# p2004dr/visual-slam

Measured on AMD Instinct MI355X. Metric: frames/sec (extract+match+pose) at 640×480, 2000 ORB, 1/2/4/8 MI355X, higher is better.
Workload: dtype u8

## Files before the change

visual-slam_amd/csrc/twoview_kernels.hip:

```cpp
#include <cmath>

#include "common.h"

#define TV_BLOCK 256
typedef double v4d __attribute__((ext_vector_type(4)));
#define TVF_BLOCK 512

#define TV_PARTS 4
#define TV_REC 10

struct TvWork {
    double* xn;
    float* xf;
    float* px;
    int* qidx;
    uint8_t* cbits;
    int* m;
    double* surv;
    int* n_alive;
    int* n_tasks;
    int2* task;
    unsigned long long* wkey;
    double* wE;
    unsigned long long* best;
// ... 257 lines not shown
}

__device__ __forceinline__ double sampson_fast(const double* E, double x1, double y1, double x2, double y2) {
    const double ex0 = fma(E[0], x1, fma(E[1], y1, E[2]));
    const double ex1 = fma(E[3], x1, fma(E[4], y1, E[5]));
    const double ex2 = fma(E[6], x1, fma(E[7], y1, E[8]));
    const double et0 = fma(E[0], x2, fma(E[3], y2, E[6]));
    const double et1 = fma(E[1], x2, fma(E[4], y2, E[7]));
    const double num = fma(x2, ex0, fma(y2, ex1, ex2));
    const double den = fma(ex0, ex0, fma(ex1, ex1, fma(et0, et0, et1 * et1)));
    double r = (double)__builtin_amdgcn_rcpf((float)den);
    r = fma(fma(-den, r, 1.0), r, r);
    return num * num * r;
}

__device__ inline uint64_t splitmix64(uint64_t& s) {
    uint64_t z = (s += 0x9E3779B97F4A7C15ull);
    z = (z ^ (z >> 30)) * 0xBF58476D1CE4E5B9ull;
    z = (z ^ (z >> 27)) * 0x94D049BB133111EBull;
    return z ^ (z >> 31);
}

__device__ __forceinline__ void sample8(uint64_t seed, int h, int m, int (&idx)[8]) {
    const uint32_t um = (uint32_t)m, q0 = 0xFFFFFFFFu / um, r0 = 0xFFFFFFFFu - q0 * um;
    const uint32_t M = r0 + 1u == um ? q0 + 1u : q0, c32 = r0 + 1u == um ? 0u : r0 + 1u;
    const bool small = m <= 65536;
    auto mod32 = [um, M](uint32_t x) {
        uint32_t r = x - __umulhi(x, M) * um;
        return r >= um ? r - um : r;
    };
    uint64_t s = seed + (uint64_t)(h + 1) * 0xD1B54A32D192ED03ull;
#pragma unroll
    for (int k = 0; k < 8; k++) {
        int c;
        bool dup;
        do {
            const uint64_t z = splitmix64(s);
            c = small ? (int)mod32(mod32((uint32_t)(z >> 32)) * c32 + mod32((uint32_t)z)) : (int)(z % (uint64_t)um);
            dup = false;
#pragma unroll
            for (int j = 0; j < k; j++) dup |= idx[j] == c;
        } while (dup);
        idx[k] = c;
    }
}

__device__ bool eight_point(const double* pts , double* E) {
    double M[9][8];
#pragma unroll
    for (int k = 0; k < 8; k++) {
        double x1 = pts[k * 4], y1 = pts[k * 4 + 1], x2 = pts[k * 4 + 2], y2 = pts[k * 4 + 3];
        M[0][k] = x2 * x1; M[1][k] = x2 * y1; M[2][k] = x2;
        M[3][k] = y2 * x1; M[4][k] = y2 * y1; M[5][k] = y2;
        M[6][k] = x1;      M[7][k] = y1;      M[8][k] = 1.0;
    }
    double beta[8];
    bool ok = true;
#pragma unroll
    for (int k = 0; k < 8; k++) {
        double nrm2 = 0;
#pragma unroll
        for (int i = k; i < 9; i++) nrm2 += M[i][k] * M[i][k];
        double nrm = sqrt(nrm2);
        ok = ok && (nrm > 1e-13);
        double alpha = M[k][k] >= 0 ? -nrm : nrm;
        double v0 = M[k][k] - alpha;
        M[k][k] = v0;
        double vtv = nrm2 - 2.0 * alpha * (v0 + alpha) + alpha * alpha;
        vtv = vtv > 0 ? vtv : 1.0;
        beta[k] = 2.0 / vtv;
#pragma unroll
        for (int j = k + 1; j < 8; j++) {
            double dot = 0;
#pragma unroll
            for (int i = k; i < 9; i++) dot += M[i][k] * M[i][j];
            dot *= beta[k];
#pragma unroll
            for (int i = k; i < 9; i++) M[i][j] -= dot * M[i][k];
        }
    }
    double n[9] = {0, 0, 0, 0, 0, 0, 0, 0, 1.0};
#pragma unroll
    for (int k = 7; k >= 0; k--) {
        double dot = 0;
#pragma unroll
        for (int i = k; i < 9; i++) dot += M[i][k] * n[i];
        dot *= beta[k];
#pragma unroll
        for (int i = k; i < 9; i++) n[i] -= dot * M[i][k];
    }
    double nn = 0;
#pragma unroll
    for (int j = 0; j < 9; j++) nn += n[j] * n[j];
    nn = 1.0 / sqrt(nn);
#pragma unroll
    for (int j = 0; j < 9; j++) E[j] = n[j] * nn;
    return ok;
}

__device__ __forceinline__ double tv_thr(const TwoViewArgs& a, const TvWork& w, int pair) {
    return a.model ? a.thr_px * w.norm[(size_t)pair * 8] : a.thr_px / ((a.K[0] + a.K[4]) / 2.0);
}

__device__ bool project_rank2(double* F) {
    double v[3];
    if (!smallest_right3(F, v)) return false;
    for (int i = 0; i < 3; i++) {
        const double fv = F[i * 3] * v[0] + F[i * 3 + 1] * v[1] + F[i * 3 + 2] * v[2];
        for (int j = 0; j < 3; j++) F[i * 3 + j] -= fv * v[j];
    }
    return true;
}

__device__ void tv_hartley(const TwoViewArgs& a, const TvWork& w, int pair, int m) {
    __shared__ double s_h[TV_BLOCK / 64][5];
    __shared__ double s_nrm[5];
    const int tid = threadIdx.x;
    const float* px = w.px + (size_t)pair * a.cap * 4;
    double* xn = w.xn + (size_t)pair * a.cap * 4;
    __syncthreads();
    double acc[4] = {0, 0, 0, 0};
    for (int i = tid; i < m; i += TV_BLOCK)
        for (int k = 0; k < 4; k++) acc[k] += (double)px[4 * i + k];
    for (int k = 0; k < 4; k++) {
        for (int o = 32; o > 0; o >>= 1) acc[k] += __shfl_xor(acc[k], o, 64);
        if ((tid & 63) == 0) s_h[tid >> 6][k] = acc[k];
    }
    __syncthreads();
    if (tid < 4) s_nrm[1 + tid] = (s_h[0][tid] + s_h[1][tid] + s_h[2][tid] + s_h[3][tid]) / (double)max(m, 1);
    __syncthreads();
    const double c1x = s_nrm[1], c1y = s_nrm[2], c2x = s_nrm[3], c2y = s_nrm[4];
    double dsum = 0;
    for (int i = tid; i < m; i += TV_BLOCK) {
        const double a1 = (double)px[4 * i] - c1x, b1 = (double)px[4 * i + 1] - c1y, a2 = (double)px[4 * i + 2] - c2x, b2 = (double)px[4 * i + 3] - c2y;
        dsum += sqrt(a1 * a1 + b1 * b1) + sqrt(a2 * a2 + b2 * b2);
    }
    for (int o = 32; o > 0; o >>= 1) dsum += __shfl_xor(dsum, o, 64);
    if ((tid & 63) == 0) s_h[tid >> 6][4] = dsum;
    __syncthreads();
    if (tid == 0) {
        const double mean = (s_h[0][4] + s_h[1][4] + s_h[2][4] + s_h[3][4]) / (2.0 * (double)max(m, 1));
        s_nrm[0] = mean > 1e-12 ? 1.4142135623730951 / mean : 1.0;
        double* o = w.norm + (size_t)pair * 8;
        o[0] = s_nrm[0]; o[1] = c1x; o[2] = c1y; o[3] = c2x; o[4] = c2y;
    }
    __syncthreads();
    const double sc = s_nrm[0];
    for (int i = tid; i < m; i += TV_BLOCK) {
        xn[4 * i] = sc * ((double)px[4 * i] - c1x); xn[4 * i + 1] = sc * ((double)px[4 * i + 1] - c1y);
        xn[4 * i + 2] = sc * ((double)px[4 * i + 2] - c2x); xn[4 * i + 3] = sc * ((double)px[4 * i + 3] - c2y);
    }
}

__device__ void tv_f32_copy(const TwoViewArgs& a, const TvWork& w, int pair, int m) {
    __shared__ float s_mx[TV_BLOCK / 64];
    const int tid = threadIdx.x;
    const double* xn = w.xn + (size_t)pair * a.cap * 4;
    float* xf = w.xf + (size_t)pair * a.cap * 4;
    __syncthreads();
    float mx = 1.0f;
    for (int i = tid; i < 4 * m; i += TV_BLOCK) {
        const float v = (float)xn[i];
        xf[i] = v;
        mx = fmaxf(mx, fabsf(v));
    }
    for (int o = 32; o > 0; o >>= 1) mx = fmaxf(mx, __shfl_xor(mx, o, 64));
    if ((tid & 63) == 0) s_mx[tid >> 6] = mx;
    __syncthreads();
    if (tid == 0) w.norm[(size_t)pair * 8 + 5] = (double)fmaxf(fmaxf(s_mx[0], s_mx[1]), fmaxf(s_mx[2], s_mx[3])) * 1.0000002;
}

__global__ __launch_bounds__(TV_BLOCK) void k_tv_prep(TwoViewArgs a, TvWork w) {
    const int pair = blockIdx.x, tid = threadIdx.x;
    __shared__ int s_w[TV_BLOCK / 64];
    __shared__ int s_base;
    const double fx = a.K[0], fy = a.K[4], cx = a.K[2], cy = a.K[5];
    double* xn = w.xn + (size_t)pair * a.cap * 4;
    float* px = w.px + (size_t)pair * a.cap * 4;
    int* qidx = w.qidx + (size_t)pair * a.cap;
    if (tid == 0) {
        s_base = 0; w.best[pair] = ~0ull; w.n_alive[pair] = 0; if (pair == 0) *w.n_tasks = 0;
        *(unsigned*)&w.norm[(size_t)pair * 8 + 6] = 0x7F800000u;
    }
    for (int j = tid; j < (a.n_hyp + 63) / 64; j += TV_BLOCK) w.wkey[(size_t)pair * ((a.n_hyp + 63) / 64) + j] = ~0ull;
    __syncthreads();
    if (a.d_p1) {
        int m = a.m_fixed;
        for (int i = tid; i < m; i += TV_BLOCK) {
            float u1 = a.d_p1[(size_t)pair * m * 2 + 2 * i], v1 = a.d_p1[(size_t)pair * m * 2 + 2 * i + 1];
            float u2 = a.d_p2[(size_t)pair * m * 2 + 2 * i], v2 = a.d_p2[(size_t)pair * m * 2 + 2 * i + 1];
            px[4 * i] = u1; px[4 * i + 1] = v1; px[4 * i + 2] = u2; px[4 * i + 3] = v2;
            xn[4 * i] = ((double)u1 - cx) / fx; xn[4 * i + 1] = ((double)v1 - cy) / fy;
            xn[4 * i + 2] = ((double)u2 - cx) / fx; xn[4 * i + 3] = ((double)v2 - cy) / fy;
            qidx[i] = i;
        }
        if (tid == 0) w.m[pair] = m;
        if (a.model) tv_hartley(a, w, pair, m);
        tv_f32_copy(a, w, pair, m);
        return;
    }
    const int qfr = a.d_qf ? a.d_qf[pair] : pair, tfr = a.d_tf ? a.d_tf[pair] : pair + 1;
    const mo_keypoint* k1 = a.d_kps + (size_t)qfr * a.cap;
    const mo_keypoint* k2 = a.d_kps + (size_t)tfr * a.cap;
    if (a.d_sel) {
        const int m = min(a.d_sel_n[pair], a.cap);
        const int32_t* sl = a.d_sel + (size_t)pair * a.cap * 2;
        for (int o = tid; o < m; o += TV_BLOCK) {
            const int i = sl[2 * o], j = sl[2 * o + 1];
            float u1 = k1[i].x, v1 = k1[i].y, u2 = k2[j].x, v2 = k2[j].y;
            px[4 * o] = u1; px[4 * o + 1] = v1; px[4 * o + 2] = u2; px[4 * o + 3] = v2;
            xn[4 * o] = ((double)u1 - cx) / fx; xn[4 * o + 1] = ((double)v1 - cy) / fy;
            xn[4 * o + 2] = ((double)u2 - cx) / fx; xn[4 * o + 3] = ((double)v2 - cy) / fy;
            qidx[o] = i;
        }
        if (tid == 0) w.m[pair] = m;
        if (a.model) tv_hartley(a, w, pair, m);
        tv_f32_copy(a, w, pair, m);
        return;
    }
    const int nq = min(a.d_counts[qfr], a.cap);
    const int32_t* midx = a.d_match_idx + (size_t)pair * a.cap * 2;
    const uint8_t* pass = a.d_match_pass + (size_t)pair * a.cap;
    for (int base = 0; base < nq; base += TV_BLOCK) {
        int i = base + tid;
        bool ok = i < nq && pass[i] && (!a.need_two || midx[2 * i + 1] >= 0);
        unsigned long long bal = __ballot(ok);
        int lane = tid & 63, wv = tid >> 6;
        int wpre = __popcll(bal & ((1ull << lane) - 1ull));
        if (lane == 0) s_w[wv] = __popcll(bal);
        __syncthreads();
        int off = s_base;
        for (int k = 0; k < wv; k++) off += s_w[k];
        if (ok) {
            int o = off + wpre;
            int j = midx[2 * i];
            float u1 = k1[i].x, v1 = k1[i].y, u2 = k2[j].x, v2 = k2[j].y;
            px[4 * o] = u1; px[4 * o + 1] = v1; px[4 * o + 2] = u2; px[4 * o + 3] = v2;
            xn[4 * o] = ((double)u1 - cx) / fx; xn[4 * o + 1] = ((double)v1 - cy) / fy;
            xn[4 * o + 2] = ((double)u2 - cx) / fx; xn[4 * o + 3] = ((double)v2 - cy) / fy;
            qidx[o] = i;
        }
        __syncthreads();
        if (tid == 0) s_base += s_w[0] + s_w[1] + s_w[2] + s_w[3];
        __syncthreads();
    }
    const int m = s_base;
    if (tid == 0) w.m[pair] = m;
    if (a.model) tv_hartley(a, w, pair, m);
    tv_f32_copy(a, w, pair, m);
}


#ifndef TV_FIRST_NUM
#define TV_FIRST_NUM 2
#endif
__device__ __forceinline__ int tv_first(int m, int num) { return min(m, max(32, (m * num + 7) >> 3)); }

__device__ __forceinline__ int tv_part_len(int m) { return (m + TV_PARTS - 1) / TV_PARTS; }
__device__ __forceinline__ double tv_cost_part(const double* E, const double* xn, int i0, int i1, double thr2) {
    typedef const __attribute__((address_space(4))) double* cdp;
    const cdp pts = (cdp)(uintptr_t)xn;
    double s = 0.0;
#pragma unroll 4
    for (int i = i0; i < i1; i++) s += fmin(sampson_fast(E, pts[4 * i], pts[4 * i + 1], pts[4 * i + 2], pts[4 * i + 3]), thr2);
    return s;
}
__device__ __forceinline__ double tv_combine(const double (&P)[TV_PARTS]) { return (P[0] + P[1]) + (P[2] + P[3]); }
__device__ __forceinline__ double tv_cost_lane(const double* E, const double* xn, int m, double thr2) {
    const int q = tv_part_len(m);
    double P[TV_PARTS];
    for (int k = 0; k < TV_PARTS; k++) P[k] = tv_cost_part(E, xn, min(m, k * q), min(m, (k + 1) * q), thr2);
    return tv_combine(P);
}

__global__ __launch_bounds__(TV_BLOCK) void k_tv_hyp(TwoViewArgs a, TvWork w, int staged, int first_num) {
    __shared__ unsigned long long s_best[TV_BLOCK / 64];
    const int pair = blockIdx.y, hb = blockIdx.x, tid = threadIdx.x;
    const int h = hb * TV_BLOCK + tid;
    const int m = w.m[pair];
    if (m < 8) return;
    const double* xn = w.xn + (size_t)pair * a.cap * 4;
    const double thr = tv_thr(a, w, pair);
    const double thr2 = thr * thr;
    double E[9];
    bool valid = h < a.n_hyp;
    if (valid) {
        int idx[8];
        sample8(a.seed + ((uint64_t)pair + a.pair_base) * 0x632BE59BD9B4E019ull, h, m, idx);
        double pts[32];
        for (int k = 0; k < 8; k++)
            for (int j = 0; j < 4; j++) pts[k * 4 + j] = xn[(size_t)idx[k] * 4 + j];
        valid = eight_point(pts, E) && (a.model ? project_rank2(E) : project_essential(E));
    }
    if (!valid) for (int j = 0; j < 9; j++) E[j] = 0.0;
    const int lane = tid & 63, wv = tid >> 6;
    const size_t ntask_max = (size_t)((a.n_hyp + 63) / 64);
    unsigned long long key = ~0ull;
    if (!staged) {
        const double cost = valid ? tv_cost_lane(E, xn, m, thr2) : 0.0;
        if (valid && cost == cost) key = ((unsigned long long)__float_as_uint((float)cost) << 32) | (unsigned long long)(unsigned)h;
        const unsigned long long own = key;
        for (int o = 32; o > 0; o >>= 1) {
            unsigned long long other = __shfl_xor(key, o, 64);
            key = other < key ? other : key;
        }
        if (lane == 0) s_best[wv] = key;
        __syncthreads();
        for (int k = 0; k < TV_BLOCK / 64; k++) key = s_best[k] < key ? s_best[k] : key;
        if (key != ~0ull && own == key) {
            double* bE = w.wE + ((size_t)pair * ntask_max + hb) * 9;
            for (int j = 0; j < 9; j++) bE[j] = E[j];
            w.wkey[(size_t)pair * ntask_max + hb] = key;
            atomicMin(&w.best[pair], key);
        }
        return;
    }
    typedef const __attribute__((address_space(4))) float* cfp;
    const cfp pf = (cfp)(uintptr_t)(w.xf + (size_t)pair * a.cap * 4);
    const int F = tv_first(m, first_num);
    const float X = (float)w.norm[(size_t)pair * 8 + 5];
    float lb = 0.0f;
    if (valid && X < 1e6f) {
        float e[9], s1 = 0.0f;
        for (int j = 0; j < 9; j++) { e[j] = (float)E[j]; s1 += fabsf(e[j]); }
        s1 *= 1.000001f;
        const float ae = 4e-7f * X * s1, delta = 2e-6f * X * X * s1, cden = 4004.0f * ae * ae;
        const float thr2f = __uint_as_float(__float_as_uint((float)thr2) - 1u);
#pragma unroll 4
        for (int i = 0; i < F; i++) {
            const float x1 = pf[4 * i], y1 = pf[4 * i + 1], x2 = pf[4 * i + 2], y2 = pf[4 * i + 3];
            const float ex0 = fmaf(e[0], x1, fmaf(e[1], y1, e[2]));
            const float ex1 = fmaf(e[3], x1, fmaf(e[4], y1, e[5]));
            const float ex2 = fmaf(e[6], x1, fmaf(e[7], y1, e[8]));
            const float et0 = fmaf(e[0], x2, fmaf(e[3], y2, e[6]));
            const float et1 = fmaf(e[1], x2, fmaf(e[4], y2, e[7]));
            const float r = fmaf(x2, ex0, fmaf(y2, ex1, ex2));
            const float den = fmaf(ex0, ex0, fmaf(ex1, ex1, fmaf(et0, et0, et1 * et1)));
            const float rl = fmaxf(fabsf(r) - delta, 0.0f);
            const float t = rl * rl * __builtin_amdgcn_rcpf(fmaf(den, 1.0011f, cden));
            lb += fminf(t, thr2f);
        }
        lb *= 0.9999f;
        if (!(lb >= 0.0f)) lb = 0.0f;
    }
    if (valid) key = ((unsigned long long)__float_as_uint(lb) << 32) | (unsigned long long)(unsigned)h;
    const unsigned long long own = key;
    for (int o = 32; o > 0; o >>= 1) {
        unsigned long long other = __shfl_xor(key, o, 64);
        key = other < key ? other : key;
    }
    if (lane == 0) s_best[wv] = key;
    __syncthreads();
    for (int k = 0; k < TV_BLOCK / 64; k++) key = s_best[k] < key ? s_best[k] : key;
    if (key == ~0ull) return;
    __shared__ double s_cand[9];
    __shared__ double s_sum[TV_BLOCK / 64];
    __shared__ unsigned s_bound;
    if (own == key)
        for (int j = 0; j < 9; j++) s_cand[j] = E[j];
    __syncthreads();
    {
        double Ec[9];
        for (int j = 0; j < 9; j++) Ec[j] = s_cand[j];
        double tot = 0.0;
        for (int i = tid; i < m; i += TV_BLOCK)
            tot += fmin(sampson_fast(Ec, xn[4 * i], xn[4 * i + 1], xn[4 * i + 2], xn[4 * i + 3]), thr2);
        for (int o = 32; o > 0; o >>= 1) tot += __shfl_xor(tot, o, 64);
        if (lane == 0) s_sum[wv] = tot;
    }
    __syncthreads();
    if (tid == 0) {
        double total = 0.0;
        for (int k = 0; k < TV_BLOCK / 64; k++) total += s_sum[k];
        unsigned bound = total == total ? __float_as_uint((float)total) + 2u : 0x7F800000u;
        const unsigned seen = atomicMin((unsigned*)&w.norm[(size_t)pair * 8 + 6], bound);
        s_bound = min(bound, seen);
    }
    __syncthreads();
    __shared__ int s_wcnt[TV_BLOCK / 64];
    __shared__ int s_gbase;
    const bool alive = own != ~0ull && __float_as_uint(lb) <= s_bound;
    const unsigned long long mk = __ballot(alive);
    if (lane == 0) s_wcnt[wv] = __popcll(mk);
    __syncthreads();
    int sbase = 0, n_alive = 0;
    for (int k = 0; k < TV_BLOCK / 64; k++) { if (k < wv) sbase += s_wcnt[k]; n_alive += s_wcnt[k]; }
    if (tid == 0) s_gbase = atomicAdd(&w.n_alive[pair], n_alive);
    __syncthreads();
    if (alive) {
        double* rec = w.surv + ((size_t)pair * a.n_hyp + s_gbase + sbase + __popcll(mk & ((1ull << lane) - 1ull))) * TV_REC;
        for (int j = 0; j < 9; j++) rec[j] = E[j];
        rec[9] = __longlong_as_double((long long)h);
    }
}

__global__ __launch_bounds__(TV_BLOCK) void k_tv_tasks(TwoViewArgs a, TvWork w) {
    __shared__ int s_off[TV_BLOCK + 1];
    const int tid = threadIdx.x;
    int total = 0;
    for (int p0 = 0; p0 < a.n_pairs; p0 += TV_BLOCK) {
        const int p = p0 + tid;
        const int nt = p < a.n_pairs ? (w.n_alive[p] + 63) / 64 : 0;
        s_off[tid + 1] = nt;
        __syncthreads();
        if (tid == 0) {
            s_off[0] = total;
            for (int k = 0; k < TV_BLOCK; k++) s_off[k + 1] += s_off[k];
        }
        __syncthreads();
        for (int j = 0; j < nt; j++) w.task[s_off[tid] + j] = make_int2(p, j);
        total = s_off[TV_BLOCK];
        __syncthreads();
    }
    if (tid == 0) *w.n_tasks = total;
}

__global__ __launch_bounds__(64 * TV_PARTS) void k_tv_score(TwoViewArgs a, TvWork w, int one_pair) {
    __shared__ double s_part[TV_PARTS][64];
    const int lane = threadIdx.x & 63, part = threadIdx.x >> 6;
    if (one_pair ? (int)blockIdx.x * 64 >= w.n_alive[0] : (int)blockIdx.x >= *w.n_tasks) return;
    const int2 tk = one_pair ? make_int2(0, (int)blockIdx.x) : w.task[blockIdx.x];
    const int pair = tk.x, t0 = tk.y * 64;
    const int total = w.n_alive[pair];
    const int m = w.m[pair];
    const double thr = tv_thr(a, w, pair);
    const double thr2 = thr * thr;
    const double* xn = w.xn + (size_t)pair * a.cap * 4;
    const bool on = t0 + lane < total;
    const double* rec = w.surv + ((size_t)pair * a.n_hyp + (on ? t0 + lane : t0)) * TV_REC;
    double E[9];
    for (int j = 0; j < 9; j++) E[j] = rec[j];
    const int q = tv_part_len(m);
    s_part[part][lane] = tv_cost_part(E, xn, min(m, part * q), min(m, (part + 1) * q), thr2);
    __syncthreads();
    if (part != 0) return;
    double P[TV_PARTS];
    for (int k = 0; k < TV_PARTS; k++) P[k] = s_part[k][lane];
    const double cost = tv_combine(P);
    const unsigned h = (unsigned)__double_as_longlong(rec[9]);
    unsigned long long key = ~0ull;
    if (on && cost == cost) key = ((unsigned long long)__float_as_uint((float)cost) << 32) | (unsigned long long)h;
    const unsigned long long own = key;
    for (int o = 32; o > 0; o >>= 1) {
        unsigned long long other = __shfl_xor(key, o, 64);
        key = other < key ? other : key;
    }
    if (key != ~0ull && own == key) {
        const size_t slot = (size_t)pair * ((a.n_hyp + 63) / 64) + tk.y;
        for (int j = 0; j < 9; j++) w.wE[slot * 9 + j] = E[j];
        w.wkey[slot] = key;
        atomicMin(&w.best[pair], key);
    }
}

#define DLT_VOTE_IT 8
#define DLT_MAP_IT 32
__device__ void dlt_point(const double* P1, const double* P2, double x1, double y1, double x2, double y2, double* X, int max_it) {
    double A[16];
#pragma unroll
    for (int k = 0; k < 4; k++) {
        A[0 * 4 + k] = x1 * P1[8 + k] - P1[k];
        A[1 * 4 + k] = y1 * P1[8 + k] - P1[4 + k];
        A[2 * 4 + k] = x2 * P2[8 + k] - P2[k];
        A[3 * 4 + k] = y2 * P2[8 + k] - P2[4 + k];
    }
    double S[10];
#pragma unroll
    for (int i = 0, k = 0; i < 4; i++)
#pragma unroll
        for (int j = i; j < 4; j++, k++) S[k] = A[i] * A[j] + A[4 + i] * A[4 + j] + A[8 + i] * A[8 + j] + A[12 + i] * A[12 + j];
    X[0] = 0.5; X[1] = 0.5; X[2] = 0.5; X[3] = 0.5;
    smallest_eigvec<4>(S, X, max_it);
}

__device__ inline double block_sum(double v, double* s_red) {
    for (int o = 32; o > 0; o >>= 1) v += __shfl_xor(v, o, 64);
    __syncthreads();
    if ((threadIdx.x & 63) == 0) s_red[threadIdx.x >> 6] = v;
    __syncthreads();
    double r = 0;
    for (int k = 0; k < TVF_BLOCK / 64; k++) r += s_red[k];
    return r;
}

__device__ inline int block_sum_i(int v, int* s_red) {
    for (int o = 32; o > 0; o >>= 1) v += __shfl_xor(v, o, 64);
    __syncthreads();
    if ((threadIdx.x & 63) == 0) s_red[threadIdx.x >> 6] = v;
    __syncthreads();
    int r = 0;
    for (int k = 0; k < TVF_BLOCK / 64; k++) r += s_red[k];
    return r;
}

#include "tv_eig9.h"

__global__ __launch_bounds__(TVF_BLOCK) void k_tv_finish(TwoViewArgs a, TvWork w) {
    __shared__ double s_red[TVF_BLOCK / 64];
    __shared__ int s_redi[TVF_BLOCK / 64];
    __shared__ double s_E[9];
    __shared__ double s_P[4][12];
    __shared__ double s_Ppix[2][12];
    __shared__ int s_ok, s_win;
    const int pair = blockIdx.x, tid = threadIdx.x;
    const int m = w.m[pair];
    double* pose = a.d_pose ? a.d_pose + (size_t)pair * 12 : nullptr;
    float* Xout = a.d_points + (size_t)pair * a.cap * 3;
    uint8_t* inl_out = a.d_inlier ? a.d_inlier + (size_t)pair * a.cap : nullptr;
    uint8_t* ran_out = a.d_ransac ? a.d_ransac + (size_t)pair * a.cap : nullptr;
    const int out_n = a.d_p1 ? a.m_fixed : a.cap;
    const float qnan = __uint_as_float(0x7FC00000u);
    for (int i = tid; i < out_n; i += TVF_BLOCK) {
        Xout[3 * i] = qnan; Xout[3 * i + 1] = qnan; Xout[3 * i + 2] = qnan;
        if (inl_out) inl_out[i] = 0;
        if (ran_out) ran_out[i] = 0;
    }
    const bool given = a.d_E_in != nullptr;
    const unsigned long long best = given ? 0ull : w.best[pair];
    if (given ? m < 1 : (m < 8 || best == ~0ull)) {
        if (tid == 0) {
            a.d_n_points[pair] = 0;
            if (pose) for (int j = 0; j < 12; j++) pose[j] = __longlong_as_double(0x7FF8000000000000ll);
            if (a.d_E) for (int j = 0; j < 9; j++) a.d_E[(size_t)pair * 9 + j] = __longlong_as_double(0x7FF8000000000000ll);
        }
        return;
    }
    const double* xn = w.xn + (size_t)pair * a.cap * 4;
    const float* px = w.px + (size_t)pair * a.cap * 4;
    const int* qidx = w.qidx + (size_t)pair * a.cap;
    const double thr = tv_thr(a, w, pair);
    const double thr2 = thr * thr;
    if (given) {
        if (tid < 9) s_E[tid] = a.d_E_in[(size_t)pair * 9 + tid];
    } else {
        const int nslot = (a.n_hyp + 63) / 64;
        for (int j = tid; j < nslot; j += TVF_BLOCK)
            if (w.wkey[(size_t)pair * nslot + j] == best)
                for (int q = 0; q < 9; q++) s_E[q] = w.wE[((size_t)pair * nslot + j) * 9 + q];
    }
    __syncthreads();

    __shared__ double s_N[45], s_M[48], s_x[9];
    __shared__ double s_R[TVF_BLOCK * 9];
    __shared__ double s_tile[TVF_BLOCK / 64][256];
    __shared__ int s_stop;
    if (!given) {
    const double lo2 = thr2 / 4096.0;
    int n0;
    double tau2;
    {
        double E[9];
        for (int j = 0; j < 9; j++) E[j] = s_E[j];
        int cnt = 0;
        double sd = 0;
        for (int i = tid; i < m; i += TVF_BLOCK) {
            double d = sampson(E, xn[4 * i], xn[4 * i + 1], xn[4 * i + 2], xn[4 * i + 3]);
            if (d <= thr2) { cnt++; sd += d; }
        }
        n0 = block_sum_i(cnt, s_redi);
        double sds = block_sum(sd, s_red);
        tau2 = n0 > 0 ? fmin(fmax(9.0 * sds / n0, lo2), thr2) : thr2;
    }
    if (n0 < 8) {
        if (tid == 0) {
            a.d_n_points[pair] = 0;
            if (pose) for (int j = 0; j < 12; j++) pose[j] = __longlong_as_double(0x7FF8000000000000ll);
            if (a.d_E) for (int j = 0; j < 9; j++) a.d_E[(size_t)pair * 9 + j] = __longlong_as_double(0x7FF8000000000000ll);
        }
        return;
    }
    int c_prev = -1;
    double tau2_prev = -1.0;
    const int lane = tid & 63, wv = tid >> 6, gc = lane & 15, gk = lane >> 4;
    for (int it = 0; it < 5; it++) {
        v4d gram = {0.0, 0.0, 0.0, 0.0};
        int cnt = 0;
        double sd = 0;
        {
            double E[9];
            for (int j = 0; j < 9; j++) E[j] = s_E[j];
            for (int base = 0; base < m; base += TVF_BLOCK) {
                const int i = base + tid;
                double r[9] = {0, 0, 0, 0, 0, 0, 0, 0, 0};
                if (i < m) {
                    double x1 = xn[4 * i], y1 = xn[4 * i + 1], x2 = xn[4 * i + 2], y2 = xn[4 * i + 3];
                    double d = sampson(E, x1, y1, x2, y2);
                    if (d <= tau2) {
                        r[0] = x2 * x1; r[1] = x2 * y1; r[2] = x2; r[3] = y2 * x1; r[4] = y2 * y1; r[5] = y2;
                        r[6] = x1; r[7] = y1; r[8] = 1.0;
                        cnt++;
                        sd += d;
                    }
                }
                __syncthreads();
#pragma unroll
                for (int j = 0; j < 9; j++) s_R[tid * 9 + j] = r[j];
                __syncthreads();
#pragma unroll 4
                for (int s4 = 0; s4 < 16; s4++) {
                    const double v = gc < 9 ? s_R[(wv * 64 + 4 * s4 + gk) * 9 + gc] : 0.0;
                    gram = __builtin_amdgcn_mfma_f64_16x16x4f64(v, v, gram, 0, 0, 0);
                }
            }
        }
        const int c = block_sum_i(cnt, s_redi);
        if (c < 8 || 2 * c < n0) break;
        if (c == c_prev && tau2 == tau2_prev) break;
        c_prev = c; tau2_prev = tau2;
        const double sds = block_sum(sd, s_red);
#pragma unroll
        for (int rg = 0; rg < 4; rg++) s_tile[wv][(gk + 4 * rg) * 16 + gc] = gram[rg];
        __syncthreads();
        if (tid < 45) {
            int p = 0, q = tid;
            while (q >= 9 - p) { q -= 9 - p; p++; }
            double v = 0;
            for (int k = 0; k < TVF_BLOCK / 64; k++) v += s_tile[k][p * 16 + p + q];
            s_N[tid] = v;
        }
        __syncthreads();
        if (tid < 64) {
            if (tid < 9) {
                double en = 0;
                for (int i = 0; i < 9; i++) en += s_E[i] * s_E[i];
                s_x[tid] = s_E[tid] / sqrt(en);
            }
            tv_wave_sync();
            const bool conv = wave_smallest_eigvec9(s_N, s_M, s_x, tid);
            if (tid == 0) {
                double E[9];
                for (int i = 0; i < 9; i++) E[i] = s_x[i];
                const bool ok = conv && (a.model ? project_rank2(E) : project_essential(E));
                if (ok) for (int i = 0; i < 9; i++) s_E[i] = E[i];
                s_stop = ok ? 0 : 1;
            }
        }
        __syncthreads();
        if (s_stop) break;
        tau2 = fmin(fmax(9.0 * sds / c, lo2), thr2);
    }
    }
    __syncthreads();
    if (a.model) {
        double Fn[9];
        for (int j = 0; j < 9; j++) Fn[j] = s_E[j];
        int cnt = 0;
        for (int i = tid; i < m; i += TVF_BLOCK) {
            const bool in = sampson(Fn, xn[4 * i], xn[4 * i + 1], xn[4 * i + 2], xn[4 * i + 3]) <= thr2;
            if (in) {
                cnt++;
                if (ran_out) ran_out[qidx[i]] = 1;
                if (inl_out) inl_out[qidx[i]] = 1;
                if (a.d_P1) {
                    double Pa[12], Pb[12], X[4];
                    for (int j = 0; j < 12; j++) { Pa[j] = a.d_P1[(size_t)pair * 12 + j]; Pb[j] = a.d_P2[(size_t)pair * 12 + j]; }
                    dlt_point(Pa, Pb, (double)px[4 * i], (double)px[4 * i + 1], (double)px[4 * i + 2], (double)px[4 * i + 3], X, DLT_MAP_IT);
                    const float xf = (float)X[0], yf = (float)X[1], zf = (float)X[2], wf = (float)X[3];
                    const int o = qidx[i];
                    Xout[3 * o] = xf / wf; Xout[3 * o + 1] = yf / wf; Xout[3 * o + 2] = zf / wf;
                }
            }
        }
        const int total = block_sum_i(cnt, s_redi);
        if (tid == 0) {
            a.d_n_points[pair] = total;
            if (pose) for (int j = 0; j < 12; j++) pose[j] = __longlong_as_double(0x7FF8000000000000ll);
            if (a.d_E) {
                const double* nm = w.norm + (size_t)pair * 8;
                const double sc = nm[0];
                const double T1[9] = {sc, 0, -sc * nm[1], 0, sc, -sc * nm[2], 0, 0, 1};
                const double T2[9] = {sc, 0, -sc * nm[3], 0, sc, -sc * nm[4], 0, 0, 1};
                double A[9], F[9], nn = 0;
                for (int i = 0; i < 3; i++)
                    for (int j = 0; j < 3; j++) { double v = 0; for (int q = 0; q < 3; q++) v += Fn[i * 3 + q] * T1[q * 3 + j]; A[i * 3 + j] = v; }
                for (int i = 0; i < 3; i++)
                    for (int j = 0; j < 3; j++) { double v = 0; for (int q = 0; q < 3; q++) v += T2[q * 3 + i] * A[q * 3 + j]; F[i * 3 + j] = v; nn += v * v; }
                const double sF = fabs(F[8]) > 1e-12 * sqrt(nn) ? 1.0 / F[8] : 1.0 / sqrt(nn);
                for (int j = 0; j < 9; j++) a.d_E[(size_t)pair * 9 + j] = F[j] * sF;
            }
        }
        return;
    }
    if (tid == 0) {
        double U[9], Vm[9], sg[3], Ef[9];
        for (int i = 0; i < 9; i++) Ef[i] = s_E[i];
        s_ok = svd3_rank2(Ef, U, Vm, sg) ? 1 : 0;
        if (s_ok) {
            const double W[9] = {0, 1, 0, -1, 0, 0, 0, 0, 1};
            double UW[9], UWt[9];
            for (int i = 0; i < 3; i++)
                for (int j = 0; j < 3; j++) {
                    double s1 = 0, s2 = 0;
                    for (int q = 0; q < 3; q++) { s1 += U[i * 3 + q] * W[q * 3 + j]; s2 += U[i * 3 + q] * W[j * 3 + q]; }
                    UW[i * 3 + j] = s1; UWt[i * 3 + j] = s2;
                }
            for (int cnd = 0; cnd < 4; cnd++) {
                const double* M = (cnd & 1) ? UWt : UW;
                double sgn = cnd >= 2 ? -1.0 : 1.0;
                for (int i = 0; i < 3; i++) {
                    for (int j = 0; j < 3; j++) {
                        double s = 0;
                        for (int q = 0; q < 3; q++) s += M[i * 3 + q] * Vm[j * 3 + q];
                        s_P[cnd][i * 4 + j] = s;
                    }
                    s_P[cnd][i * 4 + 3] = sgn * U[i * 3 + 2];
                }
            }
        }
    }
    __syncthreads();
    if (!s_ok) {
        if (tid == 0) {
            a.d_n_points[pair] = 0;
            if (pose) for (int j = 0; j < 12; j++) pose[j] = __longlong_as_double(0x7FF8000000000000ll);
        }
        return;
    }
    const double P0[12] = {1, 0, 0, 0, 0, 1, 0, 0, 0, 0, 1, 0};
    const double dist = 50.0;
    int good[4] = {0, 0, 0, 0};
    uint8_t* cbits = w.cbits + (size_t)pair * a.cap;
    double E[9];
    for (int j = 0; j < 9; j++) E[j] = s_E[j];
    for (int i = tid; i < m; i += TVF_BLOCK) {
        double x1 = xn[4 * i], y1 = xn[4 * i + 1], x2 = xn[4 * i + 2], y2 = xn[4 * i + 3];
        unsigned bits = 0;
        const bool consider = given ? (!a.d_mask_in || a.d_mask_in[(size_t)pair * a.cap + qidx[i]] != 0) : sampson(E, x1, y1, x2, y2) <= thr2;
        if (consider) {
            for (int cnd = 0; cnd < 4; cnd++) {
                double Pc[12], X[4];
                for (int j = 0; j < 12; j++) Pc[j] = s_P[cnd][j];
                dlt_point(P0, Pc, x1, y1, x2, y2, X, DLT_VOTE_IT);
                bool ok = X[2] * X[3] > 0;
                double iw = 1.0 / X[3];
                double qx = X[0] * iw, qy = X[1] * iw, qz = X[2] * iw;
                ok = ok && qz < dist;
                double z2 = Pc[8] * qx + Pc[9] * qy + Pc[10] * qz + Pc[11];
                ok = ok && z2 > 0 && z2 < dist;
                if (ok) { bits |= 1u << cnd; good[cnd]++; }
            }
            bits |= 16u;
            if (ran_out) ran_out[qidx[i]] = 1;
        }
        cbits[i] = (uint8_t)bits;
    }
    int g[4];
    for (int cnd = 0; cnd < 4; cnd++) g[cnd] = block_sum_i(good[cnd], s_redi);
    if (tid == 0) {
        int win;
        if (g[0] >= g[1] && g[0] >= g[2] && g[0] >= g[3]) win = 0;
        else if (g[1] >= g[0] && g[1] >= g[2] && g[1] >= g[3]) win = 1;
        else if (g[2] >= g[0] && g[2] >= g[1] && g[2] >= g[3]) win = 2;
        else win = 3;
        s_win = win;
        for (int i = 0; i < 3; i++)
            for (int j = 0; j < 4; j++) {
                double s1 = 0, s2 = 0;
                for (int q = 0; q < 3; q++) { s1 += a.K[i * 3 + q] * P0[q * 4 + j]; s2 += a.K[i * 3 + q] * s_P[win][q * 4 + j]; }
                s_Ppix[0][i * 4 + j] = s1; s_Ppix[1][i * 4 + j] = s2;
            }
        if (pose) {
            for (int i = 0; i < 3; i++) {
                for (int j = 0; j < 3; j++) pose[i * 3 + j] = s_P[win][i * 4 + j];
                pose[9 + i] = s_P[win][i * 4 + 3];
            }
        }
        if (a.d_E) for (int j = 0; j < 9; j++) a.d_E[(size_t)pair * 9 + j] = s_E[j];
        a.d_n_points[pair] = g[win];
    }
    __syncthreads();
    const int win = s_win;
    double Pa[12], Pb[12];
    for (int j = 0; j < 12; j++) { Pa[j] = s_Ppix[0][j]; Pb[j] = s_Ppix[1][j]; }
    for (int i = tid; i < m; i += TVF_BLOCK) {
        const unsigned bits = cbits[i];
        if (!((bits >> win) & 1u)) continue;
        double X[4];
        dlt_point(Pa, Pb, (double)px[4 * i], (double)px[4 * i + 1], (double)px[4 * i + 2], (double)px[4 * i + 3], X, DLT_MAP_IT);
        float xf = (float)X[0], yf = (float)X[1], zf = (float)X[2], wf = (float)X[3];
        int o = qidx[i];
        Xout[3 * o] = xf / wf; Xout[3 * o + 1] = yf / wf; Xout[3 * o + 2] = zf / wf;
        if (inl_out) inl_out[o] = 1;
    }
}

struct TriArgs { double P1[12], P2[12]; };

__global__ void k_triangulate(TriArgs t, const float* __restrict__ p1, const float* __restrict__ p2, int n, float* __restrict__ X4) {
    int i = blockIdx.x * blockDim.x + threadIdx.x;
    if (i >= n) return;
    double X[4];
    dlt_point(t.P1, t.P2, (double)p1[2 * i], (double)p1[2 * i + 1], (double)p2[2 * i], (double)p2[2 * i + 1], X, DLT_MAP_IT);
    for (int k = 0; k < 4; k++) X4[4 * i + k] = (float)X[k];
}

int triangulate_launch(mo_ctx* c, const double* P1, const double* P2, const float* d_p1, const float* d_p2, int n, float* d_X4) {
    if (n <= 0) return MO_OK;
    TriArgs t;
    for (int i = 0; i < 12; i++) { t.P1[i] = P1[i]; t.P2[i] = P2[i]; }
    hipLaunchKernelGGL(k_triangulate, dim3((n + 127) / 128), dim3(128), 0, c->stream, t, d_p1, d_p2, n, d_X4);
    HIPCHK(c, hipGetLastError());
    return MO_OK;
}

int twoview_launch(mo_ctx* c, const TwoViewArgs& a_in) {
    if (a_in.n_pairs <= 0) return MO_OK;
    TwoViewArgs a = a_in;
    a.flags = c->flags_cur ? c->flags_cur : c->d_flags;
    if (!a.d_E_in && (a.n_hyp < 1 || a.n_hyp > (1 << 20))) return mo_fail(c, MO_ERR_ARG, "n_hyp out of range");
    size_t need = twoview_workspace_bytes(a.n_pairs, a.cap, a.n_hyp);
    int rc = c->d_tv.reserve_exact(c, need);
    if (rc) return rc;
    TvWork w = carve(c->d_tv, a.n_pairs, a.cap, a.n_hyp);
    hipLaunchKernelGGL(k_tv_prep, dim3(a.n_pairs), dim3(TV_BLOCK), 0, c->stream, a, w);
    if (a.d_E_in) {
        hipLaunchKernelGGL(k_tv_finish, dim3(a.n_pairs), dim3(TVF_BLOCK), 0, c->stream, a, w);
        HIPCHK(c, hipGetLastError());
        return MO_OK;
    }
    const int staged = a.n_hyp >= 512;
    const int first_num = TV_FIRST_NUM;
    const dim3 hyp_grid((a.n_hyp + TV_BLOCK - 1) / TV_BLOCK, a.n_pairs);
    hipLaunchKernelGGL(k_tv_hyp, hyp_grid, dim3(TV_BLOCK), 0, c->stream, a, w, staged, first_num);
    if (staged) {
        const int one_pair = a.n_pairs == 1;
        if (!one_pair) hipLaunchKernelGGL(k_tv_tasks, dim3(1), dim3(TV_BLOCK), 0, c->stream, a, w);
        hipLaunchKernelGGL(k_tv_score, dim3((unsigned)((a.n_hyp + 63) / 64) * a.n_pairs), dim3(64 * TV_PARTS), 0, c->stream, a, w, one_pair);
    }
    hipLaunchKernelGGL(k_tv_finish, dim3(a.n_pairs), dim3(TVF_BLOCK), 0, c->stream, a, w);
    HIPCHK(c, hipGetLastError());
    return MO_OK;
}
```

Before: 126,400.

## Restructure two-view prep and finish kernels for fewer barriers and finer parallelism

k_tv_prep now writes the normalized f32 copy and its running max in the same pass that gathers matches. The match compaction processes runs of 8 per thread with a wave prefix scan, and the selection path batches its loads. In k_tv_finish, the cheirality vote is split across four lanes per point, one candidate pose each, with cbits kept in shared memory when it fits. Several block-wide reductions become fused wave reductions with fewer __syncthreads, the point tiles use wave-level syncs, and the pixel projection matrices for all four candidates are precomputed in parallel. The intent is to cut serialization, barriers and global traffic in these per-pair kernels, at the cost of more code complexity and more register and shared-memory pressure.

```diff
diff --git a/visual-slam_amd/csrc/twoview_kernels.hip b/visual-slam_amd/csrc/twoview_kernels.hip
--- a/visual-slam_amd/csrc/twoview_kernels.hip
+++ b/visual-slam_amd/csrc/twoview_kernels.hip
@@ -433,8 +433,16 @@
     }
 }
 
+__device__ void tv_f32_max(const TvWork& w, int pair, float mx) {
+    __shared__ float s_mx[TV_BLOCK / 64];
+    const int tid = threadIdx.x;
+    for (int o = 32; o > 0; o >>= 1) mx = fmaxf(mx, __shfl_xor(mx, o, 64));
+    if ((tid & 63) == 0) s_mx[tid >> 6] = mx;
+    __syncthreads();
+    if (tid == 0) w.norm[(size_t)pair * 8 + 5] = (double)fmaxf(fmaxf(s_mx[0], s_mx[1]), fmaxf(s_mx[2], s_mx[3])) * 1.0000002;
+}
+
 __device__ void tv_f32_copy(const TwoViewArgs& a, const TvWork& w, int pair, int m) {
-    __shared__ float s_mx[TV_BLOCK / 64];
     const int tid = threadIdx.x;
     const double* xn = w.xn + (size_t)pair * a.cap * 4;
     float* xf = w.xf + (size_t)pair * a.cap * 4;
@@ -445,90 +453,130 @@
         xf[i] = v;
         mx = fmaxf(mx, fabsf(v));
     }
-    for (int o = 32; o > 0; o >>= 1) mx = fmaxf(mx, __shfl_xor(mx, o, 64));
-    if ((tid & 63) == 0) s_mx[tid >> 6] = mx;
-    __syncthreads();
-    if (tid == 0) w.norm[(size_t)pair * 8 + 5] = (double)fmaxf(fmaxf(s_mx[0], s_mx[1]), fmaxf(s_mx[2], s_mx[3])) * 1.0000002;
-}
+    tv_f32_max(w, pair, mx);
+}
+
+struct TvOut {
+    double* xn; float* px; float* xf; int* qidx;
+    double fx, fy, cx, cy;
+    bool f32;
+};
+__device__ __forceinline__ float tv_emit(const TvOut& t, int o, int i, float u1, float v1, float u2, float v2, float mx) {
+    t.px[4 * o] = u1; t.px[4 * o + 1] = v1; t.px[4 * o + 2] = u2; t.px[4 * o + 3] = v2;
+    const double x1 = ((double)u1 - t.cx) / t.fx, y1 = ((double)v1 - t.cy) / t.fy;
+    const double x2 = ((double)u2 - t.cx) / t.fx, y2 = ((double)v2 - t.cy) / t.fy;
+    t.xn[4 * o] = x1; t.xn[4 * o + 1] = y1; t.xn[4 * o + 2] = x2; t.xn[4 * o + 3] = y2;
+    t.qidx[o] = i;
+    if (t.f32) {
+        const float f0 = (float)x1, f1 = (float)y1, f2 = (float)x2, f3 = (float)y2;
+        t.xf[4 * o] = f0; t.xf[4 * o + 1] = f1; t.xf[4 * o + 2] = f2; t.xf[4 * o + 3] = f3;
+        mx = fmaxf(fmaxf(fmaxf(fmaxf(mx, fabsf(f0)), fabsf(f1)), fabsf(f2)), fabsf(f3));
+    }
+    return mx;
+}
+
+#define TV_RUN 8
+#define TV_SEL 4
 
 __global__ __launch_bounds__(TV_BLOCK) void k_tv_prep(TwoViewArgs a, TvWork w) {
     const int pair = blockIdx.x, tid = threadIdx.x;
     __shared__ int s_w[TV_BLOCK / 64];
-    __shared__ int s_base;
-    const double fx = a.K[0], fy = a.K[4], cx = a.K[2], cy = a.K[5];
-    double* xn = w.xn + (size_t)pair * a.cap * 4;
-    float* px = w.px + (size_t)pair * a.cap * 4;
-    int* qidx = w.qidx + (size_t)pair * a.cap;
+    TvOut t;
+    t.xn = w.xn + (size_t)pair * a.cap * 4;
+    t.px = w.px + (size_t)pair * a.cap * 4;
+    t.xf = w.xf + (size_t)pair * a.cap * 4;
+    t.qidx = w.qidx + (size_t)pair * a.cap;
+    t.fx = a.K[0]; t.fy = a.K[4]; t.cx = a.K[2]; t.cy = a.K[5];
+    t.f32 = !a.model;
     if (tid == 0) {
-        s_base = 0; w.best[pair] = ~0ull; w.n_alive[pair] = 0; if (pair == 0) *w.n_tasks = 0;
+        w.best[pair] = ~0ull; w.n_alive[pair] = 0; if (pair == 0) *w.n_tasks = 0;
         *(unsigned*)&w.norm[(size_t)pair * 8 + 6] = 0x7F800000u;
     }
     for (int j = tid; j < (a.n_hyp + 63) / 64; j += TV_BLOCK) w.wkey[(size_t)pair * ((a.n_hyp + 63) / 64) + j] = ~0ull;
-    __syncthreads();
+    float mx = 1.0f;
+    int m;
     if (a.d_p1) {
-        int m = a.m_fixed;
+        m = a.m_fixed;
         for (int i = tid; i < m; i += TV_BLOCK) {
             float u1 = a.d_p1[(size_t)pair * m * 2 + 2 * i], v1 = a.d_p1[(size_t)pair * m * 2 + 2 * i + 1];
             float u2 = a.d_p2[(size_t)pair * m * 2 + 2 * i], v2 = a.d_p2[(size_t)pair * m * 2 + 2 * i + 1];
-            px[4 * i] = u1; px[4 * i + 1] = v1; px[4 * i + 2] = u2; px[4 * i + 3] = v2;
-            xn[4 * i] = ((double)u1 - cx) / fx; xn[4 * i + 1] = ((double)v1 - cy) / fy;
-            xn[4 * i + 2] = ((double)u2 - cx) / fx; xn[4 * i + 3] = ((double)v2 - cy) / fy;
-            qidx[i] = i;
-        }
-        if (tid == 0) w.m[pair] = m;
-        if (a.model) tv_hartley(a, w, pair, m);
+            mx = tv_emit(t, i, i, u1, v1, u2, v2, mx);
+        }
+    } else {
+        const int qfr = a.d_qf ? a.d_qf[pair] : pair, tfr = a.d_tf ? a.d_tf[pair] : pair + 1;
+        const mo_keypoint* k1 = a.d_kps + (size_t)qfr * a.cap;
+        const mo_keypoint* k2 = a.d_kps + (size_t)tfr * a.cap;
+        if (a.d_sel) {
+            m = min(a.d_sel_n[pair], a.cap);
+            const int32_t* sl = a.d_sel + (size_t)pair * a.cap * 2;
+            for (int base = 0; base < m; base += TV_BLOCK * TV_SEL) {
+                int qi[TV_SEL], ti[TV_SEL];
+#pragma unroll
+                for (int k = 0; k < TV_SEL; k++) {
+                    const int o = base + k * TV_BLOCK + tid;
+                    qi[k] = o < m ? sl[2 * o] : 0;
+                    ti[k] = o < m ? sl[2 * o + 1] : 0;
+                }
+                float u1[TV_SEL], v1[TV_SEL], u2[TV_SEL], v2[TV_SEL];
+#pragma unroll
+                for (int k = 0; k < TV_SEL; k++) { u1[k] = k1[qi[k]].x; v1[k] = k1[qi[k]].y; u2[k] = k2[ti[k]].x; v2[k] = k2[ti[k]].y; }
+#pragma unroll
+                for (int k = 0; k < TV_SEL; k++) {
+                    const int o = base + k * TV_BLOCK + tid;
+                    if (o < m) mx = tv_emit(t, o, qi[k], u1[k], v1[k], u2[k], v2[k], mx);
+                }
+            }
+        } else {
+            const int nq = min(a.d_counts[qfr], a.cap);
+            const int32_t* midx = a.d_match_idx + (size_t)pair * a.cap * 2;
+            const uint8_t* pass = a.d_match_pass + (size_t)pair * a.cap;
+            const int lane = tid & 63, wv = tid >> 6;
+            m = 0;
+            for (int base = 0; base < nq; base += TV_BLOCK * TV_RUN) {
+                const int i0 = base + tid * TV_RUN;
+                uint8_t ps[TV_RUN];
+                int j0[TV_RUN], j1[TV_RUN];
+#pragma unroll
+                for (int k = 0; k < TV_RUN; k++) {
+                    const int i = i0 + k;
+                    ps[k] = i < nq ? pass[i] : (uint8_t)0;
+                    j0[k] = i < nq ? midx[2 * i] : 0;
+                    j1[k] = i < nq && a.need_two ? midx[2 * i + 1] : 0;
+                }
+                unsigned okm = 0;
+#pragma unroll
+                for (int k = 0; k < TV_RUN; k++)
+                    if (ps[k] && j1[k] >= 0) okm |= 1u << k;
+                const int cnt = __popc(okm);
+                int inc = cnt;
+#pragma unroll
+                for (int d = 1; d < 64; d <<= 1) {
+                    const int up = __shfl_up(inc, d, 64);
+                    if (lane >= d) inc += up;
+                }
+                if (lane == 63) s_w[wv] = inc;
+                __syncthreads();
+                int o = m + inc - cnt, all = 0;
+                for (int k = 0; k < TV_BLOCK / 64; k++) { if (k < wv) o += s_w[k]; all += s_w[k]; }
+                m += all;
+                float u1[TV_RUN], v1[TV_RUN], u2[TV_RUN], v2[TV_RUN];
+#pragma unroll
+                for (int k = 0; k < TV_RUN; k++) {
+                    const int i = min(i0 + k, nq - 1), j = (okm >> k) & 1u ? j0[k] : 0;
+                    u1[k] = k1[i].x; v1[k] = k1[i].y; u2[k] = k2[j].x; v2[k] = k2[j].y;
+                }
+#pragma unroll
+                for (int k = 0; k < TV_RUN; k++)
+                    if ((okm >> k) & 1u) { mx = tv_emit(t, o, i0 + k, u1[k], v1[k], u2[k], v2[k], mx); o++; }
+                if (base + TV_BLOCK * TV_RUN < nq) __syncthreads();
+            }
+        }
+    }
+    if (tid == 0) w.m[pair] = m;
+    if (a.model) {
+        tv_hartley(a, w, pair, m);
         tv_f32_copy(a, w, pair, m);
-        return;
-    }
-    const int qfr = a.d_qf ? a.d_qf[pair] : pair, tfr = a.d_tf ? a.d_tf[pair] : pair + 1;
-    const mo_keypoint* k1 = a.d_kps + (size_t)qfr * a.cap;
-    const mo_keypoint* k2 = a.d_kps + (size_t)tfr * a.cap;
-    if (a.d_sel) {
-        const int m = min(a.d_sel_n[pair], a.cap);
-        const int32_t* sl = a.d_sel + (size_t)pair * a.cap * 2;
-        for (int o = tid; o < m; o += TV_BLOCK) {
-            const int i = sl[2 * o], j = sl[2 * o + 1];
-            float u1 = k1[i].x, v1 = k1[i].y, u2 = k2[j].x, v2 = k2[j].y;
-            px[4 * o] = u1; px[4 * o + 1] = v1; px[4 * o + 2] = u2; px[4 * o + 3] = v2;
-            xn[4 * o] = ((double)u1 - cx) / fx; xn[4 * o + 1] = ((double)v1 - cy) / fy;
-            xn[4 * o + 2] = ((double)u2 - cx) / fx; xn[4 * o + 3] = ((double)v2 - cy) / fy;
-            qidx[o] = i;
-        }
-        if (tid == 0) w.m[pair] = m;
-        if (a.model) tv_hartley(a, w, pair, m);
-        tv_f32_copy(a, w, pair, m);
-        return;
-    }
-    const int nq = min(a.d_counts[qfr], a.cap);
-    const int32_t* midx = a.d_match_idx + (size_t)pair * a.cap * 2;
-    const uint8_t* pass = a.d_match_pass + (size_t)pair * a.cap;
-    for (int base = 0; base < nq; base += TV_BLOCK) {
-        int i = base + tid;
-        bool ok = i < nq && pass[i] && (!a.need_two || midx[2 * i + 1] >= 0);
-        unsigned long long bal = __ballot(ok);
-        int lane = tid & 63, wv = tid >> 6;
-        int wpre = __popcll(bal & ((1ull << lane) - 1ull));
-        if (lane == 0) s_w[wv] = __popcll(bal);
-        __syncthreads();
-        int off = s_base;
-        for (int k = 0; k < wv; k++) off += s_w[k];
-        if (ok) {
-            int o = off + wpre;
-            int j = midx[2 * i];
-            float u1 = k1[i].x, v1 = k1[i].y, u2 = k2[j].x, v2 = k2[j].y;
-            px[4 * o] = u1; px[4 * o + 1] = v1; px[4 * o + 2] = u2; px[4 * o + 3] = v2;
-            xn[4 * o] = ((double)u1 - cx) / fx; xn[4 * o + 1] = ((double)v1 - cy) / fy;
-            xn[4 * o + 2] = ((double)u2 - cx) / fx; xn[4 * o + 3] = ((double)v2 - cy) / fy;
-            qidx[o] = i;
-        }
-        __syncthreads();
-        if (tid == 0) s_base += s_w[0] + s_w[1] + s_w[2] + s_w[3];
-        __syncthreads();
-    }
-    const int m = s_base;
-    if (tid == 0) w.m[pair] = m;
-    if (a.model) tv_hartley(a, w, pair, m);
-    tv_f32_copy(a, w, pair, m);
+    } else tv_f32_max(w, pair, mx);
 }
 
 
@@ -754,16 +802,6 @@
     smallest_eigvec<4>(S, X, max_it);
 }
 
-__device__ inline double block_sum(double v, double* s_red) {
-    for (int o = 32; o > 0; o >>= 1) v += __shfl_xor(v, o, 64);
-    __syncthreads();
-    if ((threadIdx.x & 63) == 0) s_red[threadIdx.x >> 6] = v;
-    __syncthreads();
-    double r = 0;
-    for (int k = 0; k < TVF_BLOCK / 64; k++) r += s_red[k];
-    return r;
-}
-
 __device__ inline int block_sum_i(int v, int* s_red) {
     for (int o = 32; o > 0; o >>= 1) v += __shfl_xor(v, o, 64);
     __syncthreads();
@@ -776,14 +814,29 @@
 
 #include "tv_eig9.h"
 
+template <typename T> __device__ __forceinline__ T tvf_sum8(const T* s) {
+    T r = 0;
+    for (int k = 0; k < TVF_BLOCK / 64; k++) r += s[k];
+    return r;
+}
+
+__device__ __forceinline__ int tvf_vote(const int (&g)[4]) {
+    if (g[0] >= g[1] && g[0] >= g[2] && g[0] >= g[3]) return 0;
+    if (g[1] >= g[0] && g[1] >= g[2] && g[1] >= g[3]) return 1;
+    if (g[2] >= g[0] && g[2] >= g[1] && g[2] >= g[3]) return 2;
+    return 3;
+}
+
 __global__ __launch_bounds__(TVF_BLOCK) void k_tv_finish(TwoViewArgs a, TvWork w) {
-    __shared__ double s_red[TVF_BLOCK / 64];
     __shared__ int s_redi[TVF_BLOCK / 64];
+    __shared__ int s_cnt0[TVF_BLOCK / 64], s_cnt[TVF_BLOCK / 64], s_g[4][TVF_BLOCK / 64];
+    __shared__ double s_sd0[TVF_BLOCK / 64], s_sd[TVF_BLOCK / 64];
     __shared__ double s_E[9];
     __shared__ double s_P[4][12];
-    __shared__ double s_Ppix[2][12];
-    __shared__ int s_ok, s_win;
+    __shared__ double s_Ppix[5][12];
+    __shared__ int s_ok;
     const int pair = blockIdx.x, tid = threadIdx.x;
+    const int lane = tid & 63, wv = tid >> 6;
     const int m = w.m[pair];
     double* pose = a.d_pose ? a.d_pose + (size_t)pair * 12 : nullptr;
     float* Xout = a.d_points + (size_t)pair * a.cap * 3;
@@ -791,13 +844,15 @@
     uint8_t* ran_out = a.d_ransac ? a.d_ransac + (size_t)pair * a.cap : nullptr;
     const int out_n = a.d_p1 ? a.m_fixed : a.cap;
     const float qnan = __uint_as_float(0x7FC00000u);
+    const bool given = a.d_E_in != nullptr;
+    const int nslot = (a.n_hyp + 63) / 64;
+    const unsigned long long best = given ? 0ull : w.best[pair];
+    const unsigned long long key0 = !given && tid < nslot ? w.wkey[(size_t)pair * nslot + tid] : 0ull;
     for (int i = tid; i < out_n; i += TVF_BLOCK) {
         Xout[3 * i] = qnan; Xout[3 * i + 1] = qnan; Xout[3 * i + 2] = qnan;
         if (inl_out) inl_out[i] = 0;
         if (ran_out) ran_out[i] = 0;
     }
-    const bool given = a.d_E_in != nullptr;
-    const unsigned long long best = given ? 0ull : w.best[pair];
     if (given ? m < 1 : (m < 8 || best == ~0ull)) {
         if (tid == 0) {
             a.d_n_points[pair] = 0;
@@ -814,16 +869,14 @@
     if (given) {
         if (tid < 9) s_E[tid] = a.d_E_in[(size_t)pair * 9 + tid];
     } else {
-        const int nslot = (a.n_hyp + 63) / 64;
         for (int j = tid; j < nslot; j += TVF_BLOCK)
-            if (w.wkey[(size_t)pair * nslot + j] == best)
+            if ((j == tid ? key0 : w.wkey[(size_t)pair * nslot + j]) == best)
                 for (int q = 0; q < 9; q++) s_E[q] = w.wE[((size_t)pair * nslot + j) * 9 + q];
     }
     __syncthreads();
 
     __shared__ double s_N[45], s_M[48], s_x[9];
     __shared__ double s_R[TVF_BLOCK * 9];
-    __shared__ double s_tile[TVF_BLOCK / 64][256];
     __shared__ int s_stop;
     if (!given) {
     const double lo2 = thr2 / 4096.0;
@@ -838,8 +891,11 @@
             double d = sampson(E, xn[4 * i], xn[4 * i + 1], xn[4 * i + 2], xn[4 * i + 3]);
             if (d <= thr2) { cnt++; sd += d; }
         }
-        n0 = block_sum_i(cnt, s_redi);
-        double sds = block_sum(sd, s_red);
+        for (int o = 32; o > 0; o >>= 1) { cnt += __shfl_xor(cnt, o, 64); sd += __shfl_xor(sd, o, 64); }
+        if (lane == 0) { s_cnt0[wv] = cnt; s_sd0[wv] = sd; }
+        __syncthreads();
+        n0 = tvf_sum8(s_cnt0);
+        const double sds = tvf_sum8(s_sd0);
         tau2 = n0 > 0 ? fmin(fmax(9.0 * sds / n0, lo2), thr2) : thr2;
     }
     if (n0 < 8) {
@@ -852,7 +908,7 @@
     }
     int c_prev = -1;
     double tau2_prev = -1.0;
-    const int lane = tid & 63, wv = tid >> 6, gc = lane & 15, gk = lane >> 4;
+    const int gc = lane & 15, gk = lane >> 4;
     for (int it = 0; it < 5; it++) {
         v4d gram = {0.0, 0.0, 0.0, 0.0};
         int cnt = 0;
@@ -873,10 +929,11 @@
                         sd += d;
                     }
                 }
-                __syncthreads();
+                if (base + wv * 64 >= m) continue;
+                tv_wave_sync();
 #pragma unroll
                 for (int j = 0; j < 9; j++) s_R[tid * 9 + j] = r[j];
-                __syncthreads();
+                tv_wave_sync();
 #pragma unroll 4
                 for (int s4 = 0; s4 < 16; s4++) {
                     const double v = gc < 9 ? s_R[(wv * 64 + 4 * s4 + gk) * 9 + gc] : 0.0;
@@ -884,23 +941,25 @@
                 }
             }
         }
-        const int c = block_sum_i(cnt, s_redi);
+        for (int o = 32; o > 0; o >>= 1) { cnt += __shfl_xor(cnt, o, 64); sd += __shfl_xor(sd, o, 64); }
+        if (lane == 0) { s_cnt[wv] = cnt; s_sd[wv] = sd; }
+        tv_wave_sync();
+#pragma unroll
+        for (int rg = 0; rg < 4; rg++) s_R[wv * 576 + (gk + 4 * rg) * 16 + gc] = gram[rg];
+        __syncthreads();
+        const int c = tvf_sum8(s_cnt);
         if (c < 8 || 2 * c < n0) break;
         if (c == c_prev && tau2 == tau2_prev) break;
         c_prev = c; tau2_prev = tau2;
-        const double sds = block_sum(sd, s_red);
-#pragma unroll
-        for (int rg = 0; rg < 4; rg++) s_tile[wv][(gk + 4 * rg) * 16 + gc] = gram[rg];
-        __syncthreads();
-        if (tid < 45) {
-            int p = 0, q = tid;
-            while (q >= 9 - p) { q -= 9 - p; p++; }
-            double v = 0;
-            for (int k = 0; k < TVF_BLOCK / 64; k++) v += s_tile[k][p * 16 + p + q];
-            s_N[tid] = v;
-        }
-        __syncthreads();
+        const double sds = tvf_sum8(s_sd);
         if (tid < 64) {
+            if (tid < 45) {
+                int p = 0, q = tid;
+                while (q >= 9 - p) { q -= 9 - p; p++; }
+                double v = 0;
+                for (int k = 0; k < TVF_BLOCK / 64; k++) v += s_R[k * 576 + p * 16 + p + q];
+                s_N[tid] = v;
+            }
             if (tid < 9) {
                 double en = 0;
                 for (int i = 0; i < 9; i++) en += s_E[i] * s_E[i];
@@ -999,47 +1058,55 @@
     }
     const double P0[12] = {1, 0, 0, 0, 0, 1, 0, 0, 0, 0, 1, 0};
     const double dist = 50.0;
-    int good[4] = {0, 0, 0, 0};
-    uint8_t* cbits = w.cbits + (size_t)pair * a.cap;
-    double E[9];
-    for (int j = 0; j < 9; j++) E[j] = s_E[j];
-    for (int i = tid; i < m; i += TVF_BLOCK) {
-        double x1 = xn[4 * i], y1 = xn[4 * i + 1], x2 = xn[4 * i + 2], y2 = xn[4 * i + 3];
-        unsigned bits = 0;
-        const bool consider = given ? (!a.d_mask_in || a.d_mask_in[(size_t)pair * a.cap + qidx[i]] != 0) : sampson(E, x1, y1, x2, y2) <= thr2;
-        if (consider) {
-            for (int cnd = 0; cnd < 4; cnd++) {
-                double Pc[12], X[4];
-                for (int j = 0; j < 12; j++) Pc[j] = s_P[cnd][j];
-                dlt_point(P0, Pc, x1, y1, x2, y2, X, DLT_VOTE_IT);
-                bool ok = X[2] * X[3] > 0;
-                double iw = 1.0 / X[3];
-                double qx = X[0] * iw, qy = X[1] * iw, qz = X[2] * iw;
-                ok = ok && qz < dist;
-                double z2 = Pc[8] * qx + Pc[9] * qy + Pc[10] * qz + Pc[11];
-                ok = ok && z2 > 0 && z2 < dist;
-                if (ok) { bits |= 1u << cnd; good[cnd]++; }
-            }
-            bits |= 16u;
-            if (ran_out) ran_out[qidx[i]] = 1;
-        }
-        cbits[i] = (uint8_t)bits;
-    }
-    int g[4];
-    for (int cnd = 0; cnd < 4; cnd++) g[cnd] = block_sum_i(good[cnd], s_redi);
-    if (tid == 0) {
-        int win;
-        if (g[0] >= g[1] && g[0] >= g[2] && g[0] >= g[3]) win = 0;
-        else if (g[1] >= g[0] && g[1] >= g[2] && g[1] >= g[3]) win = 1;
-        else if (g[2] >= g[0] && g[2] >= g[1] && g[2] >= g[3]) win = 2;
-        else win = 3;
-        s_win = win;
+    if (tid >= TVF_BLOCK - 4) {
+        const int cd = tid - (TVF_BLOCK - 4);
         for (int i = 0; i < 3; i++)
             for (int j = 0; j < 4; j++) {
                 double s1 = 0, s2 = 0;
-                for (int q = 0; q < 3; q++) { s1 += a.K[i * 3 + q] * P0[q * 4 + j]; s2 += a.K[i * 3 + q] * s_P[win][q * 4 + j]; }
-                s_Ppix[0][i * 4 + j] = s1; s_Ppix[1][i * 4 + j] = s2;
-            }
+                for (int q = 0; q < 3; q++) { s1 += a.K[i * 3 + q] * P0[q * 4 + j]; s2 += a.K[i * 3 + q] * s_P[cd][q * 4 + j]; }
+                if (cd == 0) s_Ppix[0][i * 4 + j] = s1;
+                s_Ppix[1 + cd][i * 4 + j] = s2;
+            }
+    }
+    uint8_t* cbits = (size_t)m <= sizeof(s_R) ? (uint8_t*)s_R : w.cbits + (size_t)pair * a.cap;
+    const int cnd = tid & 3;
+    int good = 0;
+    {
+        double E[9], Pc[12];
+        for (int j = 0; j < 9; j++) E[j] = s_E[j];
+        for (int j = 0; j < 12; j++) Pc[j] = s_P[cnd][j];
+        for (int t0 = 0; t0 < 4 * m; t0 += TVF_BLOCK) {
+            const int i = (t0 + tid) >> 2;
+            unsigned bits = 0;
+            if (i < m) {
+                double x1 = xn[4 * i], y1 = xn[4 * i + 1], x2 = xn[4 * i + 2], y2 = xn[4 * i + 3];
+                const bool consider = given ? (!a.d_mask_in || a.d_mask_in[(size_t)pair * a.cap + qidx[i]] != 0) : sampson(E, x1, y1, x2, y2) <= thr2;
+                if (consider) {
+                    double X[4];
+                    dlt_point(P0, Pc, x1, y1, x2, y2, X, DLT_VOTE_IT);
+                    bool ok = X[2] * X[3] > 0;
+                    double iw = 1.0 / X[3];
+                    double qx = X[0] * iw, qy = X[1] * iw, qz = X[2] * iw;
+                    ok = ok && qz < dist;
+                    double z2 = Pc[8] * qx + Pc[9] * qy + Pc[10] * qz + Pc[11];
+                    ok = ok && z2 > 0 && z2 < dist;
+                    if (ok) { bits = 1u << cnd; good++; }
+                    bits |= 16u;
+                    if (cnd == 0 && ran_out) ran_out[qidx[i]] = 1;
+                }
+            }
+            bits |= __shfl_xor(bits, 1, 64);
+            bits |= __shfl_xor(bits, 2, 64);
+            if (i < m && cnd == 0) cbits[i] = (uint8_t)bits;
+        }
+    }
+    int g[4];
+    for (int o = 32; o >= 4; o >>= 1) good += __shfl_xor(good, o, 64);
+    if (lane < 4) s_g[lane][wv] = good;
+    __syncthreads();
+    for (int k = 0; k < 4; k++) g[k] = tvf_sum8(s_g[k]);
+    const int win = tvf_vote(g);
+    if (tid == 0) {
         if (pose) {
             for (int i = 0; i < 3; i++) {
                 for (int j = 0; j < 3; j++) pose[i * 3 + j] = s_P[win][i * 4 + j];
@@ -1049,10 +1116,8 @@
         if (a.d_E) for (int j = 0; j < 9; j++) a.d_E[(size_t)pair * 9 + j] = s_E[j];
         a.d_n_points[pair] = g[win];
     }
-    __syncthreads();
-    const int win = s_win;
     double Pa[12], Pb[12];
-    for (int j = 0; j < 12; j++) { Pa[j] = s_Ppix[0][j]; Pb[j] = s_Ppix[1][j]; }
+    for (int j = 0; j < 12; j++) { Pa[j] = s_Ppix[0][j]; Pb[j] = s_Ppix[1 + win][j]; }
     for (int i = tid; i < m; i += TVF_BLOCK) {
         const unsigned bits = cbits[i];
         if (!((bits >> win) & 1u)) continue;
```

Result: no change. 127,300, median of 6 (+0.7%).
